# sevagh/Zen

Hardware: AMD Instinct MI355X
Metric: hops/sec (1024-hop HPR, 44.1 kHz mono) (higher is better)
Workload: dtype f32

## Files before the change

zen_amd/blockrun/blockrun.hip:

```cpp
#include "../csrc/hpr_engine.h"
#include "../csrc/masks.h"
#include "blockrun_kernel.h"
#include "zen_hip_blockrun.h"

#include <atomic>
#include <cstring>

using namespace zen_hip_impl;

namespace {

std::atomic<int> g_run_len{0}, g_min_items{4096}, g_off{0};
std::atomic<unsigned long long> g_routed{0}, g_forwarded{0};

struct ProfScope {
	zen_hip_hpr* e;
	int k;
	hipEvent_t e0 = nullptr, e1 = nullptr;
	ProfScope(zen_hip_hpr* e_, int k_)
	    : e(e_)
	    , k(k_)
	{
		if (!e->prof)
			return;
		if (!e->prof_pool.empty()) {
			e0 = e->prof_pool.back().first;
			e1 = e->prof_pool.back().second;
			e->prof_pool.pop_back();
		}
		else if (hipEventCreate(&e0) != hipSuccess || hipEventCreate(&e1) != hipSuccess) {
			e0 = e1 = nullptr;
			return;
		}
		(void)hipEventRecord(e0, e->stream);
	}
	~ProfScope()
	{
		if (!e0)
			return;
		(void)hipEventRecord(e1, e->stream);
		e->prof_pending.push_back({k, e0, e1});
		e->prof_launches[k] += 1;
	}
};

int device_slots(int* slots)
{
	static std::atomic<int> cached[64];
	int dev = 0;
	ZH_HIP(hipGetDevice(&dev));
	int v = (dev >= 0 && dev < 64) ? cached[dev].load() : 0;
	if (v == 0) {
		int cus = 0;
		ZH_HIP(hipDeviceGetAttribute(&cus, hipDeviceAttributeMultiprocessorCount, dev));
		v = 3 * (cus > 0 ? cus : 1);
		if (dev >= 0 && dev < 64)
			cached[dev].store(v);
	}
	*slots = v;
	return ZEN_HIP_OK;
}

bool takes(const zen_hip_hpr* h, const float* in, size_t n_hops, size_t in_stride, const float* harm, const float* perc,
           const float* resid, size_t out_stride)
{
	if (g_off.load() || !h || !in || !perc || harm || resid || n_hops == 0)
		return false;
	if (h->causality != ZEN_HIP_TIME_CAUSAL || h->log2n != 12 || h->mf != zen_blockrun::TAPS || h->hop != (size_t)zen_blockrun::HOP
	    || h->nfft != (size_t)zen_blockrun::NFFT || h->nwin != 2 * h->hop)
		return false;
	if (!h->out_p || h->out_h || h->out_r || h->soft || h->use_sse)
		return false;
	if ((h->drain[0] | h->drain[1] | h->drain[2]) || h->rows_stale || h->run_mode || h->res_idle_ms != 0 || h->res_active || h->dbg_stamps)
		return false;
	if (!h->d_Y[0] || !h->d_blk_need || !h->d_carry[0] || !h->d_mag || n_hops > h->max_hops)
		return false;
	if (h->n_streams * n_hops < (size_t)g_min_items.load() || h->n_streams * n_hops > 0x3fffffffu)
		return false;
	int inc = 0;
	if (hard_mask_threshold(h->beta, &inc) == 0.0)
		return false;
	const size_t S = h->n_streams;
	const char *in0 = (const char*)in, *in1 = (const char*)(in + (S - 1) * in_stride + n_hops * h->hop);
	const char *o0 = (const char*)perc, *o1 = (const char*)(perc + (S - 1) * out_stride + n_hops * h->hop);
	return !(o0 < in1 && in0 < o1);
}

}

extern "C" int zen_hip_blockrun_process(zen_hip_hpr_t h, const float* in_dev, size_t n_hops, size_t in_stride, float* harm, float* perc,
                                        float* resid, size_t out_stride)
{
	if (!takes(h, in_dev, n_hops, in_stride, harm, perc, resid, out_stride)) {
		g_forwarded.fetch_add(1);
		return zen_hip_hpr_process(h, in_dev, n_hops, in_stride, harm, perc, resid, out_stride);
	}
	g_routed.fetch_add(1);
	int slots = 0;
	ZH_TRY(device_slots(&slots));
	zen_blockrun::RunArgs a;
	memset(&a, 0, sizeof(a));
	a.in = in_dev;
	a.in_stride = (long long)in_stride;
	a.tail_prev = h->d_tail[h->tail_sel];
	a.tail_next = h->d_tail[h->tail_sel ^ 1];
	a.window = h->d_window;
	a.tw = h->d_tw;
	a.mag = h->d_mag;
	a.keep_mag_rows = (int)h->W - 1;
	a.ring_rows = h->ring_rows;
	a.row0 = h->abs_frame;
	a.n_frames = (int)n_hops;
	a.n_streams = (int)h->n_streams;
	a.prev_frames = (int)h->last_frames;
	a.carry = h->d_carry[0];
	a.Y = h->d_Y[0];
	a.y_stream_stride = (long long)(h->max_hops * h->nwin);
	a.out = perc;
	a.out_stride = (long long)out_stride;
	a.need = h->d_blk_need;
	a.cola = h->cola;
	int inc = 0;
	a.thr = hard_mask_threshold(h->beta, &inc);
	a.part = zen_blockrun_partition(a.n_streams, a.n_frames, slots, g_run_len.load());
	for (int o = 0; o < 3; ++o) {
		h->ready_valid[o] = false;
		h->direct_done[o] = false;
	}
	{
		ProfScope ps(h, zen_hip_hpr::K_FUSED);
		ZH_TRY(zen_blockrun::launch_run(a, h->stream));
	}
	{
		ProfScope ps(h, zen_hip_hpr::K_FINALIZE);
		ZH_TRY(zen_blockrun::launch_fixup(a, h->stream));
	}
	h->tail_sel ^= 1;
	h->abs_frame += (long long)n_hops;
	h->last_frames = n_hops;
	return ZEN_HIP_OK;
}

extern "C" int zen_hip_blockrun_set(const char* key, int value)
{
	if (!key || value < 0)
		ZH_FAIL(ZEN_HIP_E_BAD_ARG, "blockrun_set: null key or negative value");
	if (!strcmp(key, "run_len"))
		g_run_len.store(value);
	else if (!strcmp(key, "min_items"))
		g_min_items.store(value);
	else if (!strcmp(key, "off"))
		g_off.store(value);
	else
		ZH_FAIL(ZEN_HIP_E_BAD_ARG, "blockrun_set: unknown key '%s' (run_len, min_items, off)", key);
	return ZEN_HIP_OK;
}

extern "C" int zen_hip_blockrun_stats(unsigned long long* routed, unsigned long long* forwarded)
{
	if (routed)
		*routed = g_routed.load();
	if (forwarded)
		*forwarded = g_forwarded.load();
	return ZEN_HIP_OK;
}
```

zen_amd/blockrun/blockrun_kernel.h:

```cpp
#pragma once
#include <hip/hip_runtime.h>

#include "blockrun_partition.h"

namespace zen_blockrun {

constexpr int HOP = 1024, NFFT = 4096, TAPS = 47;

struct RunArgs {
	const float* in;
	long long in_stride;
	const float* tail_prev;
	float* tail_next;
	const float* window;
	const float2* tw;
	float* mag;
	int keep_mag_rows;
	long long ring_rows, row0;
	int n_frames, n_streams, prev_frames;
	float* carry;
	float* Y;
	long long y_stream_stride;
	float* out;
	long long out_stride;
	unsigned* need;
	float cola;
	double thr;
	zen_blockrun_part part;
};

constexpr size_t LDS_BYTES_MAX = 53 * 1024;
size_t run_kernel_lds_bytes();
int launch_run(const RunArgs& a, hipStream_t stream);
int launch_fixup(const RunArgs& a, hipStream_t stream);

}
```

zen_amd/blockrun/blockrun_kernel.hip:

```cpp
#include "../csrc/common.h"
#include "../csrc/fft_dev.h"
#include "../csrc/masks.h"
#include "../csrc/median47_core.h"
#include "../csrc/median_net.h"
#include "blockrun_kernel.h"

#pragma clang fp contract(off)

namespace zen_blockrun {
namespace {

using zen_hip_impl::hard_mask_exact;
using PL = zfft::Plan<12>;
constexpr int N = PL::N, TF = PL::TF;
static_assert(N == NFFT && TF == 256 && HOP == 4 * TF, "four samples of a hop per thread");

constexpr int MID = TAPS / 2, MID_AL = 24, IMG_END = 255 * 16 + 64;
__device__ __forceinline__ int img_addr(int g) { return (g >> 4) * zm47::RSTR + (g & 15); }
constexpr int PC_WORD = 5184, PC_TAIL = 2052, EDGE_WORD = PC_WORD + PC_TAIL + 512 + 4;
static_assert((EDGE_WORD + 256) * 4 <= PL::LDS_FLOAT2 * 8, "lean layout must fit in the frame image");
constexpr int KEEP_WORD = PL::LDS_FLOAT2 * 2, CARRY_WORD = KEEP_WORD + HOP, WIN_WORD = CARRY_WORD + HOP;
constexpr size_t LDS_BYTES = (size_t)(WIN_WORD + 2 * HOP) * 4;
static_assert(LDS_BYTES <= LDS_BYTES_MAX, "three workgroups per CU");

__device__ __forceinline__ void lds_barrier()
{
	asm volatile("s_waitcnt lgkmcnt(0)\n\ts_barrier" ::: "memory");
}

struct TwGlobal32 {
	static constexpr bool PLAIN = true;
	static constexpr bool PACKED = true;
	const float2* __restrict__ p;
	__device__ __forceinline__ float2 get(int, int, int, int idx) const
	{
		return *reinterpret_cast<const float2*>(reinterpret_cast<const char*>(p) + (unsigned)(idx << 3));
	}
};

struct Spec {
	float2 S[16];
};

struct FwdInPre {
	float x[8], w[8];
	__device__ __forceinline__ float2 operator()(int, int slot) const { return make_float2(x[slot] * w[slot], 0.0f); }
};

struct FwdOut {
	Spec* r;
	int* img;
	__device__ __forceinline__ void operator()(int idx, float2 X, bool lower, int slot) const
	{
		r->S[slot] = X;
		if (lower || idx == (N >> 1)) {
			const float m = zfft::cabs_exact(X.x, X.y);
			const int key = __float_as_int(m);
			constexpr int CH = (TF / 16) * zm47::RSTR;
			const int tfl = idx - slot * TF;
			const int a0 = img_addr(tfl + MID_AL), a1 = img_addr(N - tfl + MID_AL);
			img[a0 + slot * CH] = key;
			img[(idx == 0 || idx == (N >> 1)) ? a0 + slot * CH : a1 - slot * CH] = key;
		}
	}
};

struct InvIn {
	const Spec* r;
	const int* img;
	const float* pc;
	double thr;
	__device__ __forceinline__ float2 operator()(int idx, int slot) const
	{
		const int lo = slot * TF, hi = lo + TF - 1;
		int pi;
		if (hi <= N / 2)
			pi = idx;
		else if (lo > N / 2 && hi < N - MID)
			pi = N - idx;
		else
			pi = (idx > N / 2 && idx < N - MID) ? N - idx : (idx > N / 2 ? idx - (N - 512) + PC_TAIL : idx);
		const int g0 = idx + 24 - slot * TF;
		const float mag = __int_as_float(img[(g0 >> 4) * 20 + (g0 & 15) + slot * (TF / 16) * 20]);
		const float2 z = r->S[slot];
		const float m = hard_mask_exact(pc[pi], mag + FLT_EPSILON, thr);
		return make_float2(z.x * m, z.y * m);
	}
};

struct InvOut {
	float* Y;
	float* out;
	float* carry;
	float cola;
	__device__ __forceinline__ void operator()(int idx, float2 x, bool, int slot) const
	{
		const float y = x.x * cola;
		ZH_CHK(Y + idx, 1);
		Y[idx] = y;
		if (slot < 4) {
			ZH_CHK(out + idx, 1);
			out[idx] = carry[(slot & 3) * TF] + y;
		}
		else {
			carry[(slot & 3) * TF] = y;
		}
	}
};

__global__ __launch_bounds__(256, 3) void blockrun_kernel(RunArgs a)
{
	extern __shared__ float2 lds[];
	int* img = reinterpret_cast<int*>(lds);
	float* Prow = reinterpret_cast<float*>(img + PC_WORD);
	const int tf = (int)threadIdx.x;
	float* keep = reinterpret_cast<float*>(img + KEEP_WORD) + tf;
	float* carry = reinterpret_cast<float*>(img + CARRY_WORD) + tf;
	float* win = reinterpret_cast<float*>(img + WIN_WORD) + tf;

	int s, f0, len;
	zen_blockrun_run(&a.part, (int)blockIdx.x, &s, &f0, &len);
	if (s >= a.n_streams || f0 + len > a.n_frames)
		return;
	const float* cur = a.in + (long long)s * a.in_stride + (long long)f0 * HOP;
	float* Yrow = a.Y + (long long)s * a.y_stream_stride + (long long)f0 * (2 * HOP);
	float* orow = a.out + (long long)s * a.out_stride + (long long)f0 * HOP;

	if (a.prev_frames > 0) {
		const int fc = a.prev_frames - 1 < a.n_frames - 1 ? a.prev_frames - 1 : a.n_frames - 1;
		if (fc >= f0 && fc < f0 + len) {
			const float* y = a.Y + (long long)s * a.y_stream_stride + (long long)(a.prev_frames - 1) * (2 * HOP) + HOP;
			float v[4];
#pragma unroll
			for (int i = 0; i < 4; ++i) {
				ZH_CHK(y + tf + i * TF, 1);
				v[i] = y[tf + i * TF];
			}
#pragma unroll
			for (int i = 0; i < 4; ++i) {
				ZH_CHK(a.carry + ((long long)s * HOP + tf + i * TF), 1);
				a.carry[(long long)s * HOP + tf + i * TF] = v[i];
			}
		}
	}
	float nx[4];
	{
		const float* pv = f0 > 0 ? cur - HOP : a.tail_prev + (long long)s * HOP;
		float p[4], w[8];
#pragma unroll
		for (int m = 0; m < 4; ++m) {
			ZH_CHK(pv + m * TF + tf, 1);
			ZH_CHK(cur + m * TF + tf, 1);
			p[m] = pv[m * TF + tf];
			nx[m] = cur[m * TF + tf];
		}
#pragma unroll
		for (int m = 0; m < 8; ++m) {
			ZH_CHK(a.window + m * TF + tf, 1);
			w[m] = a.window[m * TF + tf];
		}
#pragma unroll
		for (int m = 0; m < 4; ++m) {
			keep[m * TF] = p[m];
			carry[m * TF] = 0.0f;
		}
#pragma unroll
		for (int m = 0; m < 8; ++m)
			win[m * TF] = w[m];
	}
	if (tf == 0) {
		ZH_CHK(a.need + ((long long)s * a.n_frames + f0), 1);
		a.need[(long long)s * a.n_frames + f0] = 1u;
	}

	const int tf_run = tf;
	for (int k = 0; k < len; ++k) {
		const int f = f0 + k;
		int tf = tf_run, tw_off = 0;
		asm volatile("" : "+v"(tf));
		tf &= TF - 1;
		asm volatile("" : "+s"(tw_off));
		const float2* tw = a.tw + tw_off;
		float* keep = reinterpret_cast<float*>(img + KEEP_WORD) + tf;
		float* carry = reinterpret_cast<float*>(img + CARRY_WORD) + tf;
		float* win = reinterpret_cast<float*>(img + WIN_WORD) + tf;
		Spec r;
		{
			FwdInPre pre;
#pragma unroll
			for (int m = 0; m < 4; ++m) {
				pre.x[m] = keep[m * TF];
				pre.x[4 + m] = nx[m];
			}
#pragma unroll
			for (int m = 0; m < 8; ++m)
				pre.w[m] = win[m * TF];
#pragma unroll
			for (int m = 0; m < 4; ++m)
				keep[m * TF] = nx[m];
			if (f == a.n_frames - 1) {
				float* tail = a.tail_next + (long long)s * HOP;
#pragma unroll
				for (int m = 0; m < 4; ++m) {
					ZH_CHK(tail + m * TF + tf, 1);
					tail[m * TF + tf] = nx[m];
				}
			}
			FwdOut out;
			out.r = &r;
			out.img = img;
			zfft::PassRunner<12, 0, false, true, false, FwdInPre, FwdOut, false, TwGlobal32>::run(tf, lds, TwGlobal32{tw}, pre, out, true);
		}
		lds_barrier();
		if (f >= a.n_frames - a.keep_mag_rows) {
			float* mag = a.mag + (((a.row0 + f) % a.ring_rows) + (long long)s * a.ring_rows) * N;
			for (int g = tf; g < N; g += TF) {
				ZH_CHK(mag + g, 1);
				mag[g] = __int_as_float(img[img_addr(g + MID_AL)]);
			}
		}
		{
			const int v0 = img[img_addr(MID_AL)], v1 = img[img_addr(N - 1 + MID_AL)];
			for (int g = tf; g < MID_AL; g += TF)
				img[img_addr(g)] = v0;
			for (int g = N + MID_AL + tf; g < IMG_END; g += TF)
				img[img_addr(g)] = v1;
		}
		lds_barrier();
		{
			int(*edge)[64] = reinterpret_cast<int(*)[64]>(img + EDGE_WORD);
			const int lane = tf & 63, wave = __builtin_amdgcn_readfirstlane(tf >> 6);
			const int blk = wave < 2 ? tf : (lane < 32 ? 128 + lane : 192 + lane);
			zm47::Pieces pc;
			if (wave < 3)
				zm47::m47_sort_and_publish(img, edge, blk, lane, wave, tf == 0, blk == 255, pc);
			lds_barrier();
			if (wave < 3) {
				int o[16];
				zm47::m47_select(img, edge, blk, wave, pc, o);
				const int at = blk >= 224 ? PC_TAIL + (blk - 224) * 16 : blk * 16;
				if (blk <= 127 || blk >= 224) {
#pragma unroll
					for (int v = 0; v < 4; ++v)
						*reinterpret_cast<int4*>(&Prow[at + 4 * v]) = make_int4(o[4 * v], o[4 * v + 1], o[4 * v + 2], o[4 * v + 3]);
				}
				else if (blk == 128) {
					*reinterpret_cast<int4*>(&Prow[at]) = make_int4(o[0], o[1], o[2], o[3]);
				}
			}
		}
		lds_barrier();
		cur += HOP;
		if (k + 1 < len) {
#pragma unroll
			for (int m = 0; m < 4; ++m) {
				ZH_CHK(cur + m * TF + tf, 1);
				nx[m] = cur[m * TF + tf];
			}
		}
		{
			asm volatile("" : "+v"(tf));
			asm volatile("" : "+s"(tw_off));
			tf &= TF - 1;
			tw = a.tw + tw_off;
			carry = reinterpret_cast<float*>(img + CARRY_WORD) + tf;
			InvIn in;
			in.r = &r;
			in.img = img;
			in.pc = Prow;
			in.thr = a.thr;
			InvOut out;
			out.Y = Yrow;
			out.out = orow;
			out.carry = carry;
			out.cola = a.cola;
			zfft::PassRunner<12, 0, true, false, true, InvIn, InvOut, true, TwGlobal32>::run(tf, lds, TwGlobal32{tw}, in, out, true);
		}
		Yrow += 2 * HOP;
		orow += HOP;
	}
}

__global__ __launch_bounds__(256) void blockrun_fixup_kernel(RunArgs a)
{
	const long long total = (long long)a.n_streams * a.n_frames;
	const long long item = (long long)blockIdx.x * 4 + (threadIdx.x >> 6);
	const int lane = threadIdx.x & 63;
	if (item >= total)
		return;
	ZH_CHK(a.need + item, 1);
	if (!a.need[item])
		return;
	const int s = (int)(item / a.n_frames), f = (int)(item - (long long)s * a.n_frames);
	const float* Y = a.Y + (long long)s * a.y_stream_stride + (long long)f * (2 * HOP);
	const float* prev = f == 0 ? a.carry + (long long)s * HOP : Y - HOP;
	float* o = a.out + (long long)s * a.out_stride + (long long)f * HOP;
	if (((reinterpret_cast<uintptr_t>(o) | reinterpret_cast<uintptr_t>(prev) | reinterpret_cast<uintptr_t>(Y)) & 15) == 0) {
		float4 p[HOP / 256], y[HOP / 256];
#pragma unroll
		for (int i = 0; i < HOP / 256; ++i) {
			const int k = i * 256 + lane * 4;
			ZH_CHK(prev + k, 4);
			ZH_CHK(Y + k, 4);
			p[i] = *reinterpret_cast<const float4*>(prev + k);
			y[i] = *reinterpret_cast<const float4*>(Y + k);
		}
#pragma unroll
		for (int i = 0; i < HOP / 256; ++i) {
			const int k = i * 256 + lane * 4;
			ZH_CHK(o + k, 4);
			*reinterpret_cast<float4*>(o + k) = make_float4(p[i].x + y[i].x, p[i].y + y[i].y, p[i].z + y[i].z, p[i].w + y[i].w);
		}
	}
	else {
		for (int k = lane; k < HOP; k += 64) {
			ZH_CHK(o + k, 1);
			ZH_CHK(prev + k, 1);
			ZH_CHK(Y + k, 1);
			o[k] = prev[k] + Y[k];
		}
	}
	if (lane == 0)
		a.need[item] = 0u;
}

}

size_t run_kernel_lds_bytes() { return LDS_BYTES; }

int launch_run(const RunArgs& a, hipStream_t stream)
{
	const long long runs = (long long)a.n_streams * a.part.runs_per_stream;
	hipLaunchKernelGGL(blockrun_kernel, dim3((unsigned)runs), dim3(TF), LDS_BYTES, stream, a);
	ZH_HIP(hipGetLastError());
	return ZEN_HIP_OK;
}

int launch_fixup(const RunArgs& a, hipStream_t stream)
{
	const long long total = (long long)a.n_streams * a.n_frames;
	hipLaunchKernelGGL(blockrun_fixup_kernel, dim3((unsigned)((total + 3) / 4)), dim3(256), 0, stream, a);
	ZH_HIP(hipGetLastError());
	return ZEN_HIP_OK;
}

}
```

Baseline: 58.62 million.

## Specialize first radix-16 FFT pass for real input and mirror-symmetric spectrum

Replaces the generic first radix-16 pass of the forward 4096-point FFT with a hand-written real-input pass that computes only half the outputs, deriving the rest by conjugate symmetry when the host-checked twiddle table is exactly symmetric. It also stops writing the full mirrored magnitude image and instead reads the lower half with reflected indexing in the inverse stage and the magnitude export, writing only the edge columns the median filter needs. A non-symmetric fallback kernel is kept. This cuts FFT arithmetic and LDS writes in the forward pass, at the cost of more complex indexing and two kernel variants.

```diff
diff --git a/zen_amd/blockrun/blockrun.hip b/zen_amd/blockrun/blockrun.hip
--- a/zen_amd/blockrun/blockrun.hip
+++ b/zen_amd/blockrun/blockrun.hip
@@ -1,10 +1,12 @@
 #include "../csrc/hpr_engine.h"
 #include "../csrc/masks.h"
+#include "blockrun_first_pass.h"
 #include "blockrun_kernel.h"
 #include "zen_hip_blockrun.h"
 
 #include <atomic>
 #include <cstring>
+#include <vector>
 
 using namespace zen_hip_impl;
 
@@ -61,6 +63,26 @@
 	return ZEN_HIP_OK;
 }
 
+struct FirstPassTable {
+	int symmetric;
+	float2 tw16, tw8, tw3_16;
+};
+const FirstPassTable& first_pass_table()
+{
+	static const FirstPassTable t = [] {
+		constexpr int n = zen_blockrun::NFFT;
+		std::vector<float> tw(n);
+		make_twiddles(tw.data(), tw.size());
+		FirstPassTable r;
+		r.symmetric = zen_blockrun::table_is_symmetric(tw.data(), n) ? 1 : 0;
+		r.tw16 = make_float2(tw[2 * (n / 16)], tw[2 * (n / 16) + 1]);
+		r.tw8 = make_float2(tw[2 * (n / 8)], tw[2 * (n / 8) + 1]);
+		r.tw3_16 = make_float2(tw[2 * (3 * n / 16)], tw[2 * (3 * n / 16) + 1]);
+		return r;
+	}();
+	return t;
+}
+
 bool takes(const zen_hip_hpr* h, const float* in, size_t n_hops, size_t in_stride, const float* harm, const float* perc,
            const float* resid, size_t out_stride)
 {
@@ -106,6 +128,13 @@
 	a.tail_next = h->d_tail[h->tail_sel ^ 1];
 	a.window = h->d_window;
 	a.tw = h->d_tw;
+	{
+		const FirstPassTable& t = first_pass_table();
+		a.tw_symmetric = t.symmetric;
+		a.tw16 = t.tw16;
+		a.tw8 = t.tw8;
+		a.tw3_16 = t.tw3_16;
+	}
 	a.mag = h->d_mag;
 	a.keep_mag_rows = (int)h->W - 1;
 	a.ring_rows = h->ring_rows;
diff --git a/zen_amd/blockrun/blockrun_first_pass.h b/zen_amd/blockrun/blockrun_first_pass.h
--- /dev/null
+++ b/zen_amd/blockrun/blockrun_first_pass.h
@@ -0,0 +1,110 @@
+#pragma once
+#include "../csrc/fft_dev.h"
+
+#pragma clang fp contract(off)
+
+namespace zen_blockrun {
+
+inline bool table_is_symmetric(const float* tw, int n)
+{
+	const float *e1 = tw + 2 * (n / 16), *e2 = tw + 2 * (n / 8), *e3 = tw + 2 * (3 * n / 16);
+	return e2[0] == -e2[1] && e2[0] > 0.0f && e3[0] == -e1[1] && e3[1] == -e1[0];
+}
+
+template <bool PK>
+__device__ __forceinline__ float2 cmul_eighth(float c, float2 b)
+{
+	if constexpr (PK) {
+		const zfft::v2f q = (zfft::v2f){c, c} * (zfft::v2f){b.x, b.y};
+		zfft::v2f r;
+		asm("v_pk_add_f32 %0, %1, %1 op_sel:[0,1] op_sel_hi:[1,0] neg_lo:[0,0] neg_hi:[0,1]" : "=v"(r) : "v"(q));
+		return make_float2(r.x, r.y);
+	}
+	else {
+		const float qx = c * b.x, qy = c * b.y;
+		return make_float2(qx + qy, qy - qx);
+	}
+}
+
+template <bool PK, bool SYM>
+__device__ __forceinline__ void first_pass16(const float (&p)[8], float2 w1, float2 w2, float2 w3, float2 (&Y)[16])
+{
+	using zfft::cadd;
+	using zfft::cmul;
+	using zfft::csub;
+	float s[4], d[4];
+	float2 c1[4];
+#pragma unroll
+	for (int m = 0; m < 4; ++m) {
+		s[m] = p[m] + p[m + 4];
+		d[m] = p[m] - p[m + 4];
+		c1[m] = make_float2(p[m], 0.0f - p[m + 4]);
+	}
+	float S[2], D[2];
+	float2 U[2], V[2], G[2];
+#pragma unroll
+	for (int m = 0; m < 2; ++m) {
+		S[m] = s[m] + s[m + 2];
+		D[m] = s[m] - s[m + 2];
+		const float2 t = SYM ? cmul_eighth<PK>(w2.x, c1[m + 2]) : cmul<PK>(w2, c1[m + 2]);
+		U[m] = cadd<PK>(c1[m], t);
+		V[m] = csub<PK>(c1[m], t);
+		G[m] = make_float2(d[m], 0.0f - d[m + 2]);
+	}
+	Y[0] = make_float2(S[0] + S[1], 0.0f);
+	Y[8] = make_float2(S[0] - S[1], 0.0f);
+	Y[4] = make_float2(D[0], 0.0f - D[1]);
+	Y[12] = make_float2(D[0], D[1]);
+	{
+		const float2 t = cmul<PK>(w1, U[1]);
+		Y[1] = cadd<PK>(U[0], t);
+		Y[9] = csub<PK>(U[0], t);
+	}
+	{
+		const float2 t = SYM ? cmul_eighth<PK>(w2.x, G[1]) : cmul<PK>(w2, G[1]);
+		Y[2] = cadd<PK>(G[0], t);
+		Y[10] = csub<PK>(G[0], t);
+	}
+	{
+		const float2 t = cmul<PK>(make_float2(w1.y, -w1.x), V[1]);
+		Y[5] = cadd<PK>(V[0], t);
+		Y[13] = csub<PK>(V[0], t);
+	}
+	if constexpr (SYM) {
+#pragma unroll
+		for (int k = 1; k < 16; ++k)
+			if (k == 1 || k == 2 || k == 5 || k == 9 || k == 10 || k == 13)
+				Y[16 - k] = make_float2(Y[k].x, 0.0f - Y[k].y);
+	}
+	else {
+		float2 c3[4], g3[2], g7[2], g6[2];
+#pragma unroll
+		for (int m = 0; m < 4; ++m)
+			c3[m] = make_float2(p[m], 0.0f + p[m + 4]);
+		const float2 w2i = make_float2(w2.y, -w2.x), w3i = make_float2(w3.y, -w3.x);
+#pragma unroll
+		for (int m = 0; m < 2; ++m) {
+			const float2 t = cmul<PK>(w2i, c3[m + 2]);
+			g3[m] = cadd<PK>(c3[m], t);
+			g7[m] = csub<PK>(c3[m], t);
+			g6[m] = make_float2(d[m], 0.0f + d[m + 2]);
+		}
+		{
+			const float2 t = cmul<PK>(w3, g3[1]);
+			Y[3] = cadd<PK>(g3[0], t);
+			Y[11] = csub<PK>(g3[0], t);
+		}
+		{
+			const float2 t = cmul<PK>(w2i, g6[1]);
+			Y[6] = cadd<PK>(g6[0], t);
+			Y[14] = csub<PK>(g6[0], t);
+		}
+		{
+			const float2 t = cmul<PK>(w3i, g7[1]);
+			Y[7] = cadd<PK>(g7[0], t);
+			Y[15] = csub<PK>(g7[0], t);
+		}
+	}
+}
+
+}
diff --git a/zen_amd/blockrun/blockrun_kernel.h b/zen_amd/blockrun/blockrun_kernel.h
--- a/zen_amd/blockrun/blockrun_kernel.h
+++ b/zen_amd/blockrun/blockrun_kernel.h
@@ -14,6 +14,8 @@
 	float* tail_next;
 	const float* window;
 	const float2* tw;
+	int tw_symmetric;
+	float2 tw16, tw8, tw3_16;
 	float* mag;
 	int keep_mag_rows;
 	long long ring_rows, row0;
diff --git a/zen_amd/blockrun/blockrun_kernel.hip b/zen_amd/blockrun/blockrun_kernel.hip
--- a/zen_amd/blockrun/blockrun_kernel.hip
+++ b/zen_amd/blockrun/blockrun_kernel.hip
@@ -4,6 +4,7 @@
 #include "../csrc/median47_core.h"
 #include "../csrc/median_net.h"
 #include "blockrun_kernel.h"
+#include "blockrun_first_pass.h"
 
 #pragma clang fp contract(off)
 
@@ -17,6 +18,8 @@
 
 constexpr int MID = TAPS / 2, MID_AL = 24, IMG_END = 255 * 16 + 64;
 __device__ __forceinline__ int img_addr(int g) { return (g >> 4) * zm47::RSTR + (g & 15); }
+constexpr int MIR_LO = 56, MIR_HI = 39;
+static_assert(N - MIR_LO <= 16 * 254 - 24 && N / 2 + MIR_HI >= 16 * 128 + 39, "blocks 254 / 255 and 126 .. 128 read written columns");
 constexpr int PC_WORD = 5184, PC_TAIL = 2052, EDGE_WORD = PC_WORD + PC_TAIL + 512 + 4;
 static_assert((EDGE_WORD + 256) * 4 <= PL::LDS_FLOAT2 * 8, "lean layout must fit in the frame image");
 constexpr int KEEP_WORD = PL::LDS_FLOAT2 * 2, CARRY_WORD = KEEP_WORD + HOP, WIN_WORD = CARRY_WORD + HOP;
@@ -58,9 +61,11 @@
 			const int key = __float_as_int(m);
 			constexpr int CH = (TF / 16) * zm47::RSTR;
 			const int tfl = idx - slot * TF;
-			const int a0 = img_addr(tfl + MID_AL), a1 = img_addr(N - tfl + MID_AL);
-			img[a0 + slot * CH] = key;
-			img[(idx == 0 || idx == (N >> 1)) ? a0 + slot * CH : a1 - slot * CH] = key;
+			img[img_addr(tfl + MID_AL) + slot * CH] = key;
+			if (slot == 0 && tfl >= 1 && tfl <= MIR_LO)
+				img[img_addr(N - tfl + MID_AL)] = key;
+			if (slot == 7 && tfl >= TF - MIR_HI)
+				img[img_addr(N - 7 * TF - tfl + MID_AL)] = key;
 		}
 	}
 };
@@ -80,8 +85,8 @@
 			pi = N - idx;
 		else
 			pi = (idx > N / 2 && idx < N - MID) ? N - idx : (idx > N / 2 ? idx - (N - 512) + PC_TAIL : idx);
-		const int g0 = idx + 24 - slot * TF;
-		const float mag = __int_as_float(img[(g0 >> 4) * 20 + (g0 & 15) + slot * (TF / 16) * 20]);
+		const int g0 = hi <= N / 2 ? idx + 24 - slot * TF : TF + 24 - (idx - slot * TF);
+		const float mag = __int_as_float(img[(g0 >> 4) * 20 + (g0 & 15) + (hi <= N / 2 ? slot : 15 - slot) * (TF / 16) * 20]);
 		const float2 z = r->S[slot];
 		const float m = hard_mask_exact(pc[pi], mag + FLT_EPSILON, thr);
 		return make_float2(z.x * m, z.y * m);
@@ -108,7 +113,8 @@
 	}
 };
 
-__global__ __launch_bounds__(256, 3) void blockrun_kernel(RunArgs a)
+template <bool SYM>
+__device__ __forceinline__ void run_body(const RunArgs& a)
 {
 	extern __shared__ float2 lds[];
 	int* img = reinterpret_cast<int*>(lds);
@@ -209,14 +215,26 @@
 			FwdOut out;
 			out.r = &r;
 			out.img = img;
-			zfft::PassRunner<12, 0, false, true, false, FwdInPre, FwdOut, false, TwGlobal32>::run(tf, lds, TwGlobal32{tw}, pre, out, true);
+			{
+				float p[8];
+#pragma unroll
+				for (int m = 0; m < 8; ++m)
+					p[m] = pre.x[m] * pre.w[m];
+				float2 Y0[16];
+				first_pass16<true, SYM>(p, a.tw16, a.tw8, a.tw3_16, Y0);
+#pragma unroll
+				for (int c = 0; c < 16; ++c)
+					lds[PL::pad_off(tf, c * (N / 16))] = Y0[c];
+				zfft::frame_sync<TF>();
+			}
+			zfft::PassRunner<12, 1, false, true, false, FwdInPre, FwdOut, false, TwGlobal32>::run(tf, lds, TwGlobal32{tw}, pre, out, true);
 		}
 		lds_barrier();
 		if (f >= a.n_frames - a.keep_mag_rows) {
 			float* mag = a.mag + (((a.row0 + f) % a.ring_rows) + (long long)s * a.ring_rows) * N;
 			for (int g = tf; g < N; g += TF) {
 				ZH_CHK(mag + g, 1);
-				mag[g] = __int_as_float(img[img_addr(g + MID_AL)]);
+				mag[g] = __int_as_float(img[img_addr((g <= N / 2 ? g : N - g) + MID_AL)]);
 			}
 		}
 		{
@@ -281,6 +299,9 @@
 	}
 }
 
+__global__ __launch_bounds__(256, 3) void blockrun_kernel(RunArgs a) { run_body<true>(a); }
+__global__ __launch_bounds__(256, 3) void blockrun_kernel_plain_table(RunArgs a) { run_body<false>(a); }
+
 __global__ __launch_bounds__(256) void blockrun_fixup_kernel(RunArgs a)
 {
 	const long long total = (long long)a.n_streams * a.n_frames;
@@ -331,7 +352,10 @@
 int launch_run(const RunArgs& a, hipStream_t stream)
 {
 	const long long runs = (long long)a.n_streams * a.part.runs_per_stream;
-	hipLaunchKernelGGL(blockrun_kernel, dim3((unsigned)runs), dim3(TF), LDS_BYTES, stream, a);
+	if (a.tw_symmetric)
+		hipLaunchKernelGGL(blockrun_kernel, dim3((unsigned)runs), dim3(TF), LDS_BYTES, stream, a);
+	else
+		hipLaunchKernelGGL(blockrun_kernel_plain_table, dim3((unsigned)runs), dim3(TF), LDS_BYTES, stream, a);
 	ZH_HIP(hipGetLastError());
 	return ZEN_HIP_OK;
 }
```

Measured after the change: 59.79 million (median of 6 runs). 2.0% higher.
